# neeharperi/FutureDet

Hardware: AMD Instinct MI355X
Metric: sweeps/sec end-to-end (300k pts, 10-sweep voxel) (higher is better)
Workload: dtype f32

## Files before the change

### futuredet_amd/build.py

```python
import os
import subprocess
import sys

HERE = os.path.dirname(os.path.abspath(__file__))
CSRC = os.path.join(HERE, "csrc")
OUT = os.path.join(HERE, "libfuturedet_hip.so")
SOURCES = ["fd_error.hip", "fd_voxelize.hip", "fd_index.hip", "fd_spconv.hip", "fd_spconv_v2.hip", "fd_spconv_c32.hip", "fd_spconv_f32r.hip", "fd_spconv_bf16.hip", "fd_spconv_bf16win.hip", "fd_densify.hip", "fd_conv2d.hip", "fd_conv2d_f32.hip", "fd_conv2d_wino.hip", "fd_conv2d_wino_pc.hip", "fd_decode.hip", "fd_sweeps.hip", "fd_pillars.hip", "fd_forecast.hip", "fd_deform_conv.hip", "fd_spconv_grad.hip", "fd_targets.hip", "fd_pillars_grad.hip"]
EXTRA = {"fd_decode.hip": ["-ffp-contract=off", "-fno-slp-vectorize"], "fd_sweeps.hip": ["-ffp-contract=off"], "fd_forecast.hip": ["-ffp-contract=off"],
         "fd_voxelize.hip": ["-ffp-contract=off"], "fd_pillars.hip": ["-fno-slp-vectorize"], "fd_pillars_grad.hip": ["-fno-slp-vectorize"],
         "fd_deform_conv.hip": ["-ffp-contract=off", "-fno-slp-vectorize"],
         "fd_targets.hip": ["-ffp-contract=off", "-fno-slp-vectorize"]}


def _hipcc():
    for c in (os.environ.get("HIPCC"), "/opt/rocm/bin/hipcc", "hipcc"):
        if c and (os.path.isfile(c) or c == "hipcc"):
            return c
    return "hipcc"


def needs_build():
    if not os.path.isfile(OUT):
        return True
    t = os.path.getmtime(OUT)
    deps = [os.path.join(CSRC, f) for f in os.listdir(CSRC)] + [os.path.join(HERE, "..", "include", "futuredet_hip.h"), os.path.abspath(__file__)]
    return any(os.path.getmtime(d) > t for d in deps)


def build_locked(force=False, verbose=False):
    import fcntl

    with open(os.path.join(HERE, ".build.lock"), "w") as lk:
        fcntl.flock(lk, fcntl.LOCK_EX)
        try:
            return build(force=force, verbose=verbose)
        finally:
            fcntl.flock(lk, fcntl.LOCK_UN)


def build(force=False, verbose=False):
    if not force and not needs_build():
        return OUT
    objdir = os.path.join(HERE, "csrc", "_obj")
    os.makedirs(objdir, exist_ok=True)
    objs = []
    procs = []
    for src in SOURCES:
        obj = os.path.join(objdir, src.replace(".hip", ".o"))
        cmd = [_hipcc(), "--offload-arch=gfx950", "-O3", "-std=c++17", "-fPIC", "-Wno-unused-value", "-c",
               os.path.join(CSRC, src), "-o", obj] + EXTRA.get(src, [])
        if verbose:
            print(" ".join(cmd))
        procs.append((src, subprocess.Popen(cmd)))
        objs.append(obj)
    for src, p in procs:
        if p.wait() != 0:
            raise RuntimeError("hipcc failed on " + src)
    subprocess.check_call([_hipcc(), "--offload-arch=gfx950", "-shared", "-fPIC", "-o", OUT] + objs)
    return OUT

# ... 4 lines not shown
```

### futuredet_amd/dense_bf16.py

```python
import os

import torch

from . import hip_ops
from .nn_utils import fold_stack


USE_WINOGRAD = not os.environ.get("FD_NO_WINOGRAD")


def granule(dtype):
    return 32 if dtype == torch.bfloat16 else 16


class _Conv(object):
    def __init__(self, w_oihw, bias, stride, relu, dtype):
        self.cout, self.cin, self.ks, _ = w_oihw.shape
        self.stride, self.relu, self.dtype = stride, relu, dtype
        if self.cin % granule(dtype):
            raise ValueError("conv plan: %d input channels are not a multiple of %d" % (self.cin, granule(dtype)))
        self.wpk = hip_ops.pack_conv2d_weight(w_oihw) if dtype == torch.bfloat16 else hip_ops.pack_conv2d_weight_f32(w_oihw)
        self.bias = bias.float().contiguous() if bias is not None else None
        self.fn = hip_ops.conv2d_nhwc_bf16 if dtype == torch.bfloat16 else hip_ops.conv2d_nhwc_f32
        self.wino = (dtype == torch.float32 and self.ks == 3 and stride == 1 and USE_WINOGRAD)
        self.wpk_wino = hip_ops.pack_conv2d_weight_wino(w_oihw) if self.wino else None
        self.choice = {}

    def _run(self, choice, x, out, co_off, kw):
        kind, tile = choice
        if kind == "wino":
            return hip_ops.conv2d_wino_nhwc_f32(x, self.wpk_wino, self.bias, self.cout, self.relu, out=out, co_off=co_off, tile=tile)
        return self.fn(x, self.wpk, self.bias, self.cout, self.ks, self.stride, self.relu, out=out, co_off=co_off, tile=tile, **kw)

    def _pick(self, x, out, co_off, kw):
        key = tuple(x.shape)
        c = self.choice.get(key)
        if c is not None:
            return c
        default = ("wino", 0) if (self.wino and not kw) else ("direct", 0)
        if torch.cuda.is_current_stream_capturing():
            return default
        if out is None:
            out = self._run(default, x, None, co_off, kw)
        if default[0] == "wino":
            cands = [("wino", t) for t in range(0, hip_ops.conv2d_wino_f32_num_tiles() + 1)]
        else:
            cands = [("direct", t) for t in range(0, hip_ops.conv2d_f32_num_tiles() + 1)]
        best, best_ms = default, float("inf")
        for cand in cands:
            try:
                self._run(cand, x, out, co_off, kw)
                ms = float("inf")
                for _ in range(3):
                    e0, e1 = torch.cuda.Event(enable_timing=True), torch.cuda.Event(enable_timing=True)
                    e0.record()
                    for _ in range(4):
                        self._run(cand, x, out, co_off, kw)
                    e1.record()
                    e1.synchronize()
                    ms = min(ms, e0.elapsed_time(e1))
            except hip_ops.FutureDetHipError:
                continue
            if ms < best_ms * 0.98:
                best, best_ms = cand, ms
        self.choice[key] = best
        return best

    def __call__(self, x, out=None, co_off=0, **kw):
        if self.dtype == torch.float32:
            return self._run(self._pick(x, out, co_off, kw), x, out, co_off, kw)
        return self.fn(x, self.wpk, self.bias, self.cout, self.ks, self.stride, self.relu, out=out, co_off=co_off, **kw)


class _GroupedConv(object):

    def __init__(self, wpk, bias, counts, cin_g):
        self.wpk, self.bias, self.counts, self.cin_g = wpk, bias, counts, cin_g

    def __call__(self, x, out=None):
        return hip_ops.conv2d_grouped_nhwc_f32(x, self.wpk, self.bias, self.counts, self.cin_g, relu=False, out=out)


def _convs_from_stack(modules, dtype):
    out = []
    for f in fold_stack(modules, torch.float32, False):
        assert not f.transposed
        assert (f.weight.shape[-1] == 3 and f.padding == 1) or (f.weight.shape[-1] == 1 and f.padding == 0), \
            "only 3x3 pad 1 / 1x1 pad 0 convolutions appear in the RPN / head"
        out.append(_Conv(f.weight, f.bias, f.stride, f.relu, dtype))
    return out


class RPNPlan(object):
    def __init__(self, rpn, dtype=torch.bfloat16):
        self.dtype = dtype
        self.blocks = [_convs_from_stack(b._modules.values(), dtype) for b in rpn.blocks]
        self.start = rpn.first_up
        self.deblocks = []
        for d in rpn.deblocks:
            mods = list(d._modules.values())
            f = fold_stack(mods, torch.float32, False)[0]
            if f.transposed:
                k = f.weight.shape[-1]
                assert f.stride == k and f.padding == 0
                if dtype == torch.float32 and f.weight.shape[1] % 4 == 0 and f.weight.shape[0] % 16 == 0:
                    w = f.weight.permute(2, 3, 1, 0).reshape(-1, f.weight.shape[0])[:, :, None, None].contiguous()
                    self.deblocks.append(("shuffle", k, (hip_ops.pack_conv2d_weight_f32(w), f.bias.float().contiguous(), f.relu), f.weight.shape[1]))
                    continue
                subs = [(_Conv(f.weight[:, :, dy, dx].t().contiguous()[:, :, None, None], f.bias, 1, f.relu, dtype), dy, dx)
                        for dy in range(k) for dx in range(k)]
                self.deblocks.append(("up", k, subs, f.weight.shape[1]))
            elif f.weight.shape[-1] == 1:
                assert f.stride == 1 and f.padding == 0
                self.deblocks.append(("conv", 1, _Conv(f.weight, f.bias, 1, f.relu, dtype), f.weight.shape[0]))
            else:
                k = f.weight.shape[-1]
                assert f.stride == k and f.padding == 0
                w = f.weight.permute(0, 2, 3, 1).reshape(f.weight.shape[0], -1)[:, :, None, None].contiguous()
                self.deblocks.append(("down", k, _Conv(w, f.bias, 1, f.relu, dtype), f.weight.shape[0]))
        self.cout_total = sum(d[3] for d in self.deblocks)

    def __call__(self, x):
        ups = None
        co = 0
        for i, stack in enumerate(self.blocks):
            for conv in stack:
                x = conv(x)
            j = i - self.start
            if j >= 0:
                kind, k, op, cout = self.deblocks[j]
                B, H, W, C = x.shape
                Ho, Wo = (H // k, W // k) if kind == "down" else (H * k, W * k)
                if ups is None:
# ... 26 lines not shown
        if head.bev_map:
            st = fold_stack(head.bev_conv, torch.float32, False)
            g = granule(dtype)
            w0 = st[0].weight
            self.bev_cin = w0.shape[1]
            w0 = torch.cat([w0, torch.zeros((w0.shape[0], (-w0.shape[1]) % g) + tuple(w0.shape[2:]), dtype=w0.dtype, device=w0.device)], dim=1)
            self.bev = [_Conv(w0, st[0].bias, 1, True, dtype)] + [_Conv(f.weight, f.bias, f.stride, f.relu, dtype) for f in st[1:]]
        self.ff = bool(head.forecast_feature)
        self.tasks = []
        self.adapt = []
        self.pre = []
        for ti, task in enumerate(head.tasks):
            if self.ff:
                st = fold_stack(task.forecast_conv, torch.float32, False)
                assert len(st) == 2
                w0 = st[0].weight
                if ti == 0:
                    w0 = torch.cat([w0, torch.zeros_like(w0)], dim=1)
                self.pre.append((_Conv(w0, st[0].bias, 1, True, dtype), _Conv(st[1].weight, st[1].bias, 1, True, dtype)))
            dcn = getattr(task, "task_head", None) is not None
            sep = task.task_head if dcn else task
            names = list(sep.heads)
            stacks = [list(getattr(sep, h)._modules.values()) for h in names]
            if dcn:
                names.append("hm")
                stacks.append(list(task.cls_head._modules.values()))
            firsts, finals = [], []
            for mods in stacks:
                st = fold_stack(mods, torch.float32, False)
                assert len(st) == 2
                firsts.append(st[0])
                finals.append(st[1])
            w1 = torch.cat([f.weight for f in firsts], 0)
            b1 = torch.cat([f.bias for f in firsts], 0)
            adapt = None
            if dcn:
                fc, fr = task.feature_adapt_cls, task.feature_adapt_reg
                adapt = hip_ops.pack_deform_adapt(fc.conv_adaption.weight, fr.conv_adaption.weight, fc.conv_offset.weight, fc.conv_offset.bias,
                                                  fr.conv_offset.weight, fr.conv_offset.bias, dtype == torch.bfloat16)
                cin = w1.shape[1]
                n_hm = firsts[-1].weight.shape[0]
                z = torch.zeros_like(w1)
                w1 = torch.cat([torch.cat([z[:-n_hm], w1[:-n_hm]], 1), torch.cat([w1[-n_hm:], z[-n_hm:]], 1)], 0)
                assert w1.shape[1] == 2 * cin
            hc = firsts[0].weight.shape[0]
            couts = [f.weight.shape[0] for f in finals]
            w2 = torch.zeros((sum(couts), hc * len(names), 3, 3), dtype=torch.float32, device=w1.device)
            o = 0
            for i, f in enumerate(finals):
                w2[o:o + couts[i], i * hc:(i + 1) * hc] = f.weight
                o += couts[i]
            b2 = torch.cat([f.bias for f in finals], 0)
            if dtype == torch.float32 and len(names) <= 8 and max(couts) <= 16 and hc % 16 == 0 and finals[0].weight.shape[-1] == 3:
                wg = torch.zeros((16 * len(names), hc, 3, 3), dtype=torch.float32, device=w1.device)
                bg = torch.zeros((16 * len(names),), dtype=torch.float32, device=w1.device)
                for i, f in enumerate(finals):
                    wg[16 * i:16 * i + couts[i]] = f.weight
                    bg[16 * i:16 * i + couts[i]] = f.bias
                c2 = _GroupedConv(hip_ops.pack_conv2d_weight_f32(wg), bg.contiguous(), list(couts), hc)
            else:
                c2 = _Conv(w2, b2, 1, False, dtype)
            self.tasks.append((_Conv(w1, b1, 1, True, dtype), c2, names, couts))
            self.adapt.append(adapt)

    def __call__(self, x, bev_map=None):
        if self.bev is not None:
            assert bev_map is not None, "this head has a bev_map branch"
            for conv in self.shared:
                x = conv(x)
            B, H, W, _ = x.shape
            y = torch.zeros((B, H, W, self.bev[0].cin), dtype=self.dtype, device=x.device)
            y[..., : self.bev_cin] = bev_map.permute(0, 2, 3, 1)
            for conv in self.bev:
                y = conv(y)
            x = x + y
            return self._tasks(x, None)
        for conv in self.shared[:-1]:
            x = conv(x)
        last = self.shared[-1]
        hc = last.cout
        if self.ff:
            B, H, W, _ = x.shape
            cat = [torch.empty((B, H, W, 2 * hc), dtype=self.dtype, device=x.device) for _ in range(2)]
            cat[0][..., hc:].zero_()
            last(x, out=cat[0], co_off=0)
            cat[1][..., :hc].copy_(cat[0][..., :hc])
        else:
            x = last(x)
            cat = None
        return self._tasks(x, cat)

    def _tasks(self, x, cat):
        hc = self.shared[-1].cout
        if self.ff and cat is None:
            B, H, W, _ = x.shape
            cat = [torch.empty((B, H, W, 2 * hc), dtype=self.dtype, device=x.device) for _ in range(2)]
            cat[0][..., hc:].zero_()
            cat[0][..., :hc].copy_(x)
            cat[1][..., :hc].copy_(x)
        rets = []
        zbuf = None
        for ti, (c1, c2, names, couts) in enumerate(self.tasks):
            d = HeadMaps()
            if self.ff:
                p0, p1 = self.pre[ti]
                x = p1(p0(cat[ti & 1]))
                cat[(ti + 1) & 1][..., hc:].copy_(x)
                d["feats"] = x.permute(0, 3, 1, 2)
            adapt = self.adapt[ti]
            y1 = c1(x if adapt is None else hip_ops.deform_adapt_nhwc(x, adapt[0], adapt[1], adapt[2]))
            uniform = all(tuple(t[3]) == tuple(self.tasks[0][3]) for t in self.tasks)
            if uniform:
# ... 17 lines not shown
```

### futuredet_amd/hip_ops.py

```python
import ctypes
import threading

import numpy as np
import torch

from . import lib as _lib
from .lib import DecodeCfg, FutureDetHipError, MapView, check


_raw_stream = getattr(torch._C, "_cuda_getCurrentRawStream", None)


def _stream():
    if _raw_stream is not None:
        return ctypes.c_void_p(_raw_stream(torch.cuda.current_device()))
    return ctypes.c_void_p(torch.cuda.current_stream().cuda_stream)


def _dev(t, name, dtype=None):
    if not isinstance(t, torch.Tensor) or not t.is_cuda:
        raise FutureDetHipError("%s must be a tensor on the HIP device (got %s); this path has no CPU implementation"
                                % (name, "cpu tensor" if isinstance(t, torch.Tensor) else type(t)))
    if dtype is not None and t.dtype != dtype:
        raise FutureDetHipError("%s must be %s, got %s" % (name, dtype, t.dtype))
# ... 433 lines not shown
    nbytes = L.fd_conv2d_f32_packed_weight_bytes(cout, cin, ks)
    if nbytes == 0:
        raise FutureDetHipError("fd_conv2d_f32: unsupported weight shape %s" % (tuple(w.shape),))
    host = torch.empty((nbytes,), dtype=torch.uint8)
    check(L.fd_conv2d_f32_pack_weight(ctypes.c_void_p(w.data_ptr()), cout, cin, ks, ctypes.c_void_p(host.data_ptr())),
          "fd_conv2d_f32_pack_weight")
    return host.to(dev)


def conv2d_nhwc_f32(x, wpk, bias, cout, ks, stride=1, relu=True, out=None, co_off=0, osy=1, osx=1, ooy=0, oox=0, tile=0):
    L = _lib.load()
    x = _dev(x, "x", torch.float32)
    B, H, W, cin = x.shape
    pad = 1 if ks == 3 else 0
    Ho, Wo = (H + 2 * pad - ks) // stride + 1, (W + 2 * pad - ks) // stride + 1
    if out is None:
        out = torch.empty((B, Ho * osy, Wo * osx, cout), dtype=torch.float32, device=x.device)
    _dev(out, "out", torch.float32)
    check(L.fd_conv2d_nhwc_f32(_p(x), B, H, W, cin, _p(wpk), _p(bias), cout, ks, stride, pad, int(bool(relu)), _p(out),
                               out.shape[3], co_off, osy, osx, ooy, oox, int(tile), _stream()), "fd_conv2d_nhwc_f32")
    return out


def conv2d_f32_num_tiles():
    return int(_lib.load().fd_conv2d_f32_num_tiles())


def conv2d_shuffle_nhwc_f32(x, wpk, bias, cout_sub, k, relu=True, out=None, co_off=0, tile=0):
    L = _lib.load()
    x = _dev(x, "x", torch.float32)
    B, H, W, cin = x.shape
    if out is None:
        out = torch.empty((B, H * k, W * k, cout_sub), dtype=torch.float32, device=x.device)
    _dev(out, "out", torch.float32)
    check(L.fd_conv2d_shuffle_nhwc_f32(_p(x), B, H, W, cin, _p(wpk), _p(bias), int(cout_sub), int(k), int(bool(relu)), _p(out), out.shape[3],
                                       co_off, int(tile), _stream()), "fd_conv2d_shuffle_nhwc_f32")
    return out


def conv2d_grouped_nhwc_f32(x, wpk, bias, counts, cin_g, relu=False, out=None, co_off=0, tile=0):
    L = _lib.load()
    x = _dev(x, "x", torch.float32)
    B, H, W, cin = x.shape
    groups = len(counts)
    assert cin == groups * cin_g
    if out is None:
        out = torch.empty((B, H, W, int(sum(counts))), dtype=torch.float32, device=x.device)
    _dev(out, "out", torch.float32)
    check(L.fd_conv2d_grouped_nhwc_f32(_p(x), B, H, W, groups, int(cin_g), _p(wpk), _p(bias), (ctypes.c_int * groups)(*[int(c) for c in counts]),
                                       int(bool(relu)), _p(out), out.shape[3], co_off, int(tile), _stream()), "fd_conv2d_grouped_nhwc_f32")
    return out


def pack_conv2d_weight_wino(w_oihw):
    L = _lib.load()
    dev = w_oihw.device
    w = w_oihw.detach().to("cpu", torch.float32).contiguous()
    cout, cin, ks, _ = w.shape
    nbytes = L.fd_conv2d_wino_f32_packed_weight_bytes(cout, cin) if ks == 3 else 0
    if nbytes == 0:
        raise FutureDetHipError("fd_conv2d_wino_f32: unsupported weight shape %s" % (tuple(w.shape),))
    host = torch.empty((nbytes,), dtype=torch.uint8)
    check(L.fd_conv2d_wino_f32_pack_weight(ctypes.c_void_p(w.data_ptr()), cout, cin, ctypes.c_void_p(host.data_ptr())),
          "fd_conv2d_wino_f32_pack_weight")
    return host.to(dev)


def conv2d_wino_nhwc_f32(x, wpk, bias, cout, relu=True, out=None, co_off=0, tile=0):
    L = _lib.load()
    x = _dev(x, "x", torch.float32)
    B, H, W, cin = x.shape
    if out is None:
        out = torch.empty((B, H, W, cout), dtype=torch.float32, device=x.device)
    _dev(out, "out", torch.float32)
    check(L.fd_conv2d_wino_nhwc_f32(_p(x), B, H, W, cin, _p(wpk), _p(bias), cout, int(bool(relu)), _p(out), out.shape[3], co_off, int(tile),
                                    _stream()), "fd_conv2d_wino_nhwc_f32")
    return out


def conv2d_wino_f32_num_tiles():
    return int(_lib.load().fd_conv2d_wino_f32_num_tiles())


CIRCLE_PRE_MAX = 4096


def pack_deform_adapt(w_cls, w_reg, off_w_cls, off_b_cls, off_w_reg, off_b_reg, bf16):
    L = _lib.load()
    dev = w_cls.device
    wc = w_cls.detach().to("cpu", torch.float32).contiguous()
    wr = w_reg.detach().to("cpu", torch.float32).contiguous()
    if tuple(wc.shape) != (64, 64, 3, 3) or tuple(wr.shape) != (64, 64, 3, 3):
        raise FutureDetHipError("fd_deform_adapt: conv_adaption weights must be [64, 64, 3, 3], got %s / %s" % (tuple(wc.shape), tuple(wr.shape)))
    host = torch.empty((L.fd_deform_adapt_packed_weight_bytes(int(bool(bf16))),), dtype=torch.uint8)
    check(L.fd_deform_adapt_pack_weight(ctypes.c_void_p(wc.data_ptr()), ctypes.c_void_p(wr.data_ptr()), int(bool(bf16)),
                                        ctypes.c_void_p(host.data_ptr())), "fd_deform_adapt_pack_weight")
    ow = torch.stack([off_w_cls.detach().float().reshape(72, 64), off_w_reg.detach().float().reshape(72, 64)]).contiguous()
    ob = torch.stack([off_b_cls.detach().float().reshape(72), off_b_reg.detach().float().reshape(72)]).contiguous()
    return host.to(dev), ow.to(dev), ob.to(dev)


def deform_adapt_nhwc(x, wpk, off_w=None, off_b=None, offsets=None, out=None):
    L = _lib.load()
    if x.dtype not in (torch.float32, torch.bfloat16):
        raise FutureDetHipError("x must be float32 or bfloat16, got %s" % (x.dtype,))
    x = _dev(x, "x")
# ... 380 lines not shown
```

### futuredet_amd/lib.py

```python
import ctypes
import os

_HERE = os.path.dirname(os.path.abspath(__file__))
LIB_PATH = os.environ.get("FD_LIB_PATH") or os.path.join(_HERE, "libfuturedet_hip.so")
_lib = None

c_void_p = ctypes.c_void_p
c_int = ctypes.c_int
c_i64 = ctypes.c_int64
c_size_t = ctypes.c_size_t
c_float = ctypes.c_float


class MapView(ctypes.Structure):
    _fields_ = [("data", ctypes.c_void_p), ("group_stride", ctypes.c_int64), ("channel_stride", ctypes.c_int64), ("cell_stride", ctypes.c_int64),
                ("dtype", ctypes.c_int)]


ABI_VERSION = 8


class DecodeCfg(ctypes.Structure):
    _fields_ = [("H", c_int), ("W", c_int), ("out_size_factor", c_float), ("voxel_x", c_float), ("voxel_y", c_float),
                ("pc_x", c_float), ("pc_y", c_float), ("score_threshold", c_float), ("center_range", c_float * 6),
# ... 8 lines not shown


class ForecastBuffers(ctypes.Structure):
    _fields_ = [(n, c_void_p) for n in ("center", "quat", "velocity", "size", "fwd_idx", "fwd_ok", "bwd_idx", "bwd_ok", "match_idx", "cv_centers",
                                        "status", "traj_kind", "traj_src", "traj_first", "traj_group", "n_traj")]


class TargetsCfg(ctypes.Structure):
    _fields_ = [("H", c_int), ("W", c_int), ("T", c_int), ("n_max", c_int), ("max_objs", c_int), ("n_sets", c_int), ("n_tasks", c_int),
                ("task_classes", c_int * 16), ("radius_mult", c_int), ("min_radius", c_int), ("out_size_factor", c_float), ("voxel_x", c_float),
                ("voxel_y", c_float), ("pc_x", c_float), ("pc_y", c_float), ("gaussian_overlap", ctypes.c_double)]


SIGNATURES = {
    "fd_abi_version": (c_int, []),
    "fd_last_error": (ctypes.c_char_p, []),
    "fd_tuning_set": (c_int, [ctypes.c_char_p, c_int]),
    "fd_voxelize_workspace_bytes": (c_size_t, [c_i64, c_i64]),
    "fd_voxelize": (c_int, [c_void_p, c_i64, c_void_p, c_int, c_void_p, c_void_p, c_int, c_i64, c_int, c_void_p, c_void_p, c_int,
                            c_void_p, c_int, c_void_p, c_void_p, c_void_p, c_size_t, c_void_p]),
    "fd_index_num_cols": (c_i64, [c_int, c_int, c_int]),
    "fd_index_workspace_bytes": (c_size_t, [c_i64]),
    "fd_index_mark": (c_int, [c_void_p, c_void_p, c_i64, c_int, c_int, c_int, c_int, c_void_p, c_void_p]),
    "fd_index_downsample": (c_int, [c_void_p, c_int, c_int, c_int, c_int, c_void_p, c_void_p, c_void_p, c_void_p, c_void_p]),
    "fd_index_scan": (c_int, [c_void_p, c_i64, c_void_p, c_void_p, c_void_p, c_size_t, c_void_p]),
    "fd_index_coords": (c_int, [c_void_p, c_void_p, c_int, c_int, c_int, c_int, c_void_p, c_void_p]),
    "fd_index_lookup": (c_int, [c_void_p, c_void_p, c_int, c_int, c_int, c_int, c_void_p, c_void_p, c_i64, c_void_p, c_void_p]),
    "fd_rows_permute": (c_int, [c_void_p, c_int, c_void_p, c_void_p, c_i64, c_void_p, c_int, c_int, c_void_p]),
    "fd_rulebook": (c_int, [c_void_p, c_void_p, c_int, c_int, c_int, c_int, c_void_p, c_i64, c_void_p, c_i64, c_int, c_void_p, c_void_p,
                            c_void_p, c_void_p, c_void_p]),
    "fd_spconv_packed_weight_bytes": (c_size_t, [c_int, c_int, c_int, c_int]),
    "fd_spconv_pack_weight": (c_int, [c_void_p, c_int, c_int, c_int, c_int, c_void_p]),
    "fd_spconv_apply": (c_int, [c_void_p, c_i64, c_void_p, c_void_p, c_void_p, c_int, c_void_p, c_i64, c_void_p, c_int, c_int, c_i64,
                                c_void_p, c_i64, c_int, c_int, c_int, c_void_p, c_void_p]),
    "fd_spconv_num_ranges": (c_int, [c_i64, c_int, c_int, c_int]),
    "fd_spconv_wants_balanced_ranges": (c_int, [c_int, c_int, c_int]),
    "fd_spconv_ranges_workspace_bytes": (c_size_t, [c_i64]),
    "fd_spconv_ranges": (c_int, [c_void_p, c_i64, c_int, c_i64, c_void_p, c_int, c_void_p, c_void_p, c_size_t, c_void_p]),
    "fd_densify": (c_int, [c_void_p, c_int, c_int, c_void_p, c_void_p, c_int, c_int, c_int, c_int, c_void_p, c_int, c_i64,
                           c_i64, c_i64, c_i64, c_i64, c_void_p]),
    "fd_conv2d_packed_weight_bytes": (c_size_t, [c_int, c_int, c_int]),
    "fd_conv2d_pack_weight": (c_int, [c_void_p, c_int, c_int, c_int, c_void_p]),
    "fd_conv2d_nhwc_bf16": (c_int, [c_void_p, c_int, c_int, c_int, c_int, c_void_p, c_void_p, c_int, c_int, c_int, c_int, c_int,
                                    c_void_p, c_int, c_int, c_int, c_int, c_int, c_int, c_void_p]),
    "fd_conv2d_f32_packed_weight_bytes": (c_size_t, [c_int, c_int, c_int]),
    "fd_conv2d_f32_pack_weight": (c_int, [c_void_p, c_int, c_int, c_int, c_void_p]),
    "fd_conv2d_f32_num_tiles": (c_int, []),
    "fd_conv2d_nhwc_f32": (c_int, [c_void_p, c_int, c_int, c_int, c_int, c_void_p, c_void_p, c_int, c_int, c_int, c_int, c_int,
                                   c_void_p, c_int, c_int, c_int, c_int, c_int, c_int, c_int, c_void_p]),
    "fd_conv2d_shuffle_nhwc_f32": (c_int, [c_void_p, c_int, c_int, c_int, c_int, c_void_p, c_void_p, c_int, c_int, c_int, c_void_p, c_int, c_int, c_int,
                                           c_void_p]),
    "fd_conv2d_grouped_nhwc_f32": (c_int, [c_void_p, c_int, c_int, c_int, c_int, c_int, c_void_p, c_void_p, c_void_p, c_int, c_void_p, c_int, c_int,
                                           c_int, c_void_p]),
    "fd_conv2d_wino_f32_num_tiles": (c_int, []),
    "fd_conv2d_wino_f32_packed_weight_bytes": (c_size_t, [c_int, c_int]),
    "fd_conv2d_wino_f32_pack_weight": (c_int, [c_void_p, c_int, c_int, c_void_p]),
    "fd_conv2d_wino_nhwc_f32": (c_int, [c_void_p, c_int, c_int, c_int, c_int, c_void_p, c_void_p, c_int, c_int, c_void_p, c_int, c_int, c_int,
                                        c_void_p]),
    "fd_decode_workspace_bytes": (c_size_t, [c_int, ctypes.POINTER(DecodeCfg)]),
    "fd_centerpoint_decode": (c_int, [c_void_p, c_i64, c_void_p, c_i64, c_void_p, c_i64, c_void_p, c_i64, c_void_p, c_i64,
                                      c_int, ctypes.POINTER(DecodeCfg), c_void_p, c_void_p, c_void_p, c_void_p, c_void_p,
                                      c_size_t, c_void_p]),
    "fd_centerpoint_decode_maps": (c_int, [ctypes.POINTER(MapView)] * 5 + [c_int, ctypes.POINTER(DecodeCfg), c_void_p, c_void_p, c_void_p, c_void_p,
                                           c_void_p, c_size_t, c_void_p]),
    "fd_centerpoint_decode_packed": (c_int, [ctypes.POINTER(MapView)] * 6 + [c_int, c_int, ctypes.POINTER(DecodeCfg), c_int, c_void_p, c_void_p, c_void_p,
                                             c_void_p, c_void_p, c_void_p, c_void_p, c_void_p, c_void_p, c_void_p, c_size_t, c_void_p]),
    "fd_assemble_detections": (c_int, [c_void_p, c_void_p, c_void_p, c_void_p, ctypes.POINTER(MapView), c_int, c_int, c_int, c_void_p, c_void_p,
                                       c_void_p, c_void_p, c_void_p, c_void_p]),
    "fd_nms_workspace_bytes": (c_size_t, [c_int]),
    "fd_rotated_nms": (c_int, [c_void_p, c_int, c_float, c_void_p, c_void_p, c_void_p, c_size_t, c_void_p]),
    "fd_boxes_iou_bev": (c_int, [c_void_p, c_int, c_void_p, c_int, c_void_p, c_void_p]),
    "fd_pillar_encode": (c_int, [c_void_p, c_void_p, c_void_p, c_void_p, c_i64, c_int, c_int, c_int, c_float, c_float, c_float,
                                 c_float, c_void_p, c_void_p, c_void_p, c_int, c_void_p, c_void_p, c_void_p, c_int, c_int,
                                 c_void_p, c_int, c_void_p]),
    "fd_pillar_scatter": (c_int, [c_void_p, c_int, c_int, c_int, c_void_p, c_void_p, c_i64, c_int, c_int, c_int, c_void_p, c_int,
                                  c_i64, c_i64, c_i64, c_i64, c_int, c_void_p]),
    "fd_forecast_chains": (c_int, [c_void_p, c_void_p, c_void_p, c_void_p, c_int, c_int, ctypes.c_double, c_void_p, c_void_p,
                                   c_void_p, c_void_p, c_void_p, c_void_p, c_void_p, c_void_p]),
    "fd_det_to_global_boxes": (c_int, [c_void_p, c_int, c_void_p, c_void_p, c_void_p, c_void_p, c_void_p, c_void_p, c_void_p, c_void_p, c_void_p]),
    "fd_forecast_groups": (c_int, [c_void_p, c_int, ctypes.c_double, c_void_p, c_void_p]),
    "fd_forecast_from_detections": (c_int, [c_void_p, c_void_p, c_int, c_int, c_int, c_int, c_void_p, c_void_p, ctypes.c_double, ctypes.c_double,
                                            ctypes.POINTER(ForecastBuffers), c_void_p]),
    "fd_nearest_rows": (c_int, [c_void_p, c_int, c_void_p, c_int, c_int, c_void_p, c_void_p]),
    "fd_index_pyramid": (c_int, [c_void_p, c_void_p, c_i64, c_int, c_int, ctypes.POINTER(IndexLevel), c_void_p, c_void_p, c_size_t,
                                 c_void_p]),
    "fd_index_pyramid_coords": (c_int, [c_int, c_int, ctypes.POINTER(IndexLevel), c_void_p]),
    "fd_rows_place": (c_int, [c_void_p, c_void_p, c_int, c_int, c_int, c_int, c_void_p, c_void_p, c_i64, c_void_p, c_int, c_void_p,
                              c_int, c_int, c_void_p]),
    "fd_sweep_assemble_workspace_bytes": (c_size_t, [c_i64]),
    "fd_sweep_assemble": (c_int, [c_void_p, c_int, c_int, c_i64, c_void_p, c_int, c_float, c_void_p, c_void_p, c_void_p,
                                  c_size_t, c_void_p]),
    "fd_deform_adapt_packed_weight_bytes": (c_size_t, [c_int]),
    "fd_deform_adapt_pack_weight": (c_int, [c_void_p, c_void_p, c_int, c_void_p]),
    "fd_deform_adapt_nhwc": (c_int, [c_void_p, c_int, c_int, c_int, c_int, c_int, c_void_p, c_void_p, c_void_p, c_void_p, c_void_p, c_void_p]),
    "fd_spconv_wgrad_workspace_bytes": (c_size_t, [c_int, c_i64, c_int, c_int]),
    "fd_spconv_wgrad": (c_int, [c_void_p, c_i64, c_void_p, c_void_p, c_i64, c_int, c_i64, c_void_p, c_int, c_int, c_void_p, c_void_p, c_size_t,
                                c_void_p]),
    "fd_rulebook_transpose": (c_int, [c_void_p, c_i64, c_int, c_i64, c_void_p, c_i64, c_void_p, c_i64, c_void_p]),
    "fd_spconv_pack_weight_device": (c_int, [c_void_p, c_int, c_int, c_int, c_int, c_void_p, c_void_p]),
    "fd_dense_gather": (c_int, [c_void_p, c_i64, c_i64, c_i64, c_i64, c_int, c_void_p, c_i64, c_void_p, c_int, c_void_p, c_void_p]),
    "fd_pillar_train_workspace_bytes": (c_size_t, [c_i64, c_int]),
    "fd_pillar_train_forward": (c_int, [c_void_p, c_void_p, c_void_p, c_i64, c_int, c_int, c_int, c_float, c_float, c_float, c_float,
                                        c_void_p, c_void_p, c_void_p, c_int, c_float, c_void_p, c_void_p, c_void_p, c_int, c_float,
                                        c_void_p, c_void_p, c_void_p, c_void_p, c_void_p, c_void_p, c_size_t, c_void_p]),
    "fd_pillar_train_backward": (c_int, [c_void_p, c_void_p, c_void_p, c_i64, c_int, c_int, c_int, c_float, c_float, c_float, c_float,
                                         c_void_p, c_void_p, c_void_p, c_int, c_void_p, c_void_p, c_void_p, c_int, c_void_p,
# ... 35 lines not shown
```

### include/futuredet_hip.h

```cpp
#ifndef FUTUREDET_HIP_H
#define FUTUREDET_HIP_H

#include <stddef.h>
#include <stdint.h>

#ifdef __cplusplus
extern "C" {
#endif

#define FD_OK 0
#define FD_EINVAL (-1)
#define FD_EWORKSPACE (-2)
#define FD_ELAUNCH (-3)

typedef void *fd_stream_t;

int fd_abi_version(void);
const char *fd_last_error(void);
int fd_tuning_set(const char *name, int value);

size_t fd_voxelize_workspace_bytes(int64_t n_points, int64_t max_voxels);
int fd_voxelize(const float *points, int64_t n_points, const int32_t *n_points_dev, int ndim, const float *range6_host,
                const float *voxel_size3_host, int max_points, int64_t max_voxels, int batch_idx,
                float *out_voxels, float *out_mean, int mean_stride, int32_t *out_coors, int coor_cols,
// ... 2 lines not shown

int64_t fd_index_num_cols(int B, int H, int W);
size_t fd_index_workspace_bytes(int64_t num_cols);
int fd_index_mark(const int32_t *coords , const int32_t *n_dev ,
                  int64_t n_max, int B, int D, int H, int W, uint64_t *words, fd_stream_t stream);
int fd_index_downsample(const uint64_t *in_words, int B, int D, int H, int W, const int *ksize3,
                        const int *stride3, const int *pad3, uint64_t *out_words, fd_stream_t stream);
int fd_index_scan(const uint64_t *words, int64_t num_cols, int32_t *prefix, int32_t *n_active_dev,
                  void *workspace, size_t workspace_bytes, fd_stream_t stream);
int fd_index_coords(const uint64_t *words, const int32_t *prefix, int B, int D, int H, int W,
                    int32_t *coords , fd_stream_t stream);
int fd_index_lookup(const uint64_t *words, const int32_t *prefix, int B, int D, int H, int W,
                    const int32_t *coords_in, const int32_t *n_dev, int64_t n_max, int32_t *row_of,
                    fd_stream_t stream);
int fd_rows_permute(const float *src, int c_src, const int32_t *row_of, const int32_t *n_dev, int64_t n_max,
                    void *dst, int c_dst, int dst_bf16, fd_stream_t stream);
int fd_rulebook(const uint64_t *in_words, const int32_t *in_prefix, int B, int Din, int Hin, int Win,
                const int32_t *out_coords, int64_t out_rows, const int32_t *n_out_dev, int64_t nbr_stride, int fill_tail, const int *ksize3,
                const int *stride3, const int *pad3, int32_t *nbr, fd_stream_t stream);

size_t fd_spconv_packed_weight_bytes(int K, int cin, int cout, int dtype);
int fd_spconv_pack_weight(const float *w_kio_host, int K, int cin, int cout, int dtype, void *wpacked_host);
int fd_spconv_apply(const void *in_feats, int64_t n_in, const void *wpacked, const float *bias, const void *residual,
                    int relu, const int32_t *nbr, int64_t nbr_stride, const int32_t *ranges ,
                    int n_ranges, int K, int64_t n_out, const int32_t *n_out_dev ,
                    int64_t n_expected ,
                    int cin, int cout, int dtype, void *out_feats, fd_stream_t stream);
int fd_spconv_num_ranges(int64_t n_out, int cin, int cout, int dtype);
int fd_spconv_wants_balanced_ranges(int cin, int cout, int dtype);
size_t fd_spconv_ranges_workspace_bytes(int64_t n_out);
int fd_spconv_ranges(const int32_t *nbr, int64_t nbr_stride, int K, int64_t n_out, const int32_t *n_out_dev, int n_ranges,
                     int32_t *ranges , void *workspace, size_t workspace_bytes, fd_stream_t stream);

int fd_densify(const void *feats, int c, int dtype, const uint64_t *words, const int32_t *prefix, int B, int D,
               int H, int W, void *out, int out_dtype, int64_t stride_b, int64_t stride_c, int64_t stride_y,
               int64_t stride_x, int64_t n_rows ,
               fd_stream_t stream);

size_t fd_conv2d_packed_weight_bytes(int cout, int cin, int ks);
int fd_conv2d_pack_weight(const float *w_oihw_host, int cout, int cin, int ks, void *wpacked_host);
int fd_conv2d_nhwc_bf16(const void *x, int B, int H, int W, int cin, const void *wpacked, const float *bias, int cout,
                        int ks, int stride, int pad, int relu, void *y, int cout_total, int co_off, int osy, int osx,
                        int ooy, int oox, fd_stream_t stream);
size_t fd_conv2d_f32_packed_weight_bytes(int cout, int cin, int ks);
int fd_conv2d_f32_pack_weight(const float *w_oihw_host, int cout, int cin, int ks, void *wpacked_host);
int fd_conv2d_f32_num_tiles(void);
int fd_conv2d_nhwc_f32(const float *x, int B, int H, int W, int cin, const void *wpacked, const float *bias, int cout, int ks,
                       int stride, int pad, int relu, float *y, int cout_total, int co_off, int osy, int osx, int ooy, int oox,
                       int tile , fd_stream_t stream);
int fd_conv2d_shuffle_nhwc_f32(const float *x, int B, int H, int W, int cin, const void *wpacked, const float *bias, int cout_sub, int k,
                               int relu, float *y, int cout_total, int co_off, int tile, fd_stream_t stream);
int fd_conv2d_grouped_nhwc_f32(const float *x, int B, int H, int W, int groups, int cin_g, const void *wpacked, const float *bias,
                               const int *counts_host, int relu, float *y, int cout_total, int co_off, int tile, fd_stream_t stream);
int fd_conv2d_wino_f32_num_tiles(void);
size_t fd_conv2d_wino_f32_packed_weight_bytes(int cout, int cin);
int fd_conv2d_wino_f32_pack_weight(const float *w_oihw_host, int cout, int cin, void *wpacked_host);
int fd_conv2d_wino_nhwc_f32(const float *x, int B, int H, int W, int cin, const void *wpacked, const float *bias, int cout, int relu,
                            float *y, int cout_total, int co_off, int tile , fd_stream_t stream);

typedef struct fd_decode_cfg {
    int H, W;
    float out_size_factor, voxel_x, voxel_y, pc_x, pc_y;
    float score_threshold;
    float center_range[6];
    float nms_iou_threshold;
    int nms_pre_max, nms_post_max;
    int hm_channels;
    int nms_kind;
    int n_radius;
    float circle_radius[16];
} fd_decode_cfg;

typedef struct fd_map_view {
    const void *data;
    int64_t group_stride, channel_stride, cell_stride;
    int dtype;
} fd_map_view;

size_t fd_decode_workspace_bytes(int G, const fd_decode_cfg *cfg);
int fd_centerpoint_decode_maps(const fd_map_view *hm, const fd_map_view *reg, const fd_map_view *height, const fd_map_view *dim,
                               const fd_map_view *rot, int G, const fd_decode_cfg *cfg_host, float *out_boxes7, float *out_scores,
                               int32_t *out_cell, int32_t *out_count, void *workspace, size_t workspace_bytes, fd_stream_t stream);
int fd_assemble_detections(const float *boxes7, const float *scores, const int32_t *cell, const int32_t *count, const fd_map_view *vel,
                           int B, int post_max, int S, const int32_t *step_group, const int32_t *step_vel_channel,
                           const int32_t *step_label, float *packed, int32_t *counts_out, fd_stream_t stream);
int fd_centerpoint_decode_packed(const fd_map_view *hm, const fd_map_view *reg, const fd_map_view *height, const fd_map_view *dim,
                                 const fd_map_view *rot, const fd_map_view *vel, int G, int B, const fd_decode_cfg *cfg_host, int S,
                                 const int32_t *step_group, const int32_t *step_vel_channel, const int32_t *step_label, float *out_boxes7,
                                 float *out_scores, int32_t *out_cell, int32_t *out_count, float *packed, int32_t *counts_out, void *workspace,
                                 size_t workspace_bytes, fd_stream_t stream);
int fd_centerpoint_decode(const float *hm, int64_t hm_gstride, const float *reg, int64_t reg_gstride,
                          const float *height, int64_t height_gstride, const float *dim, int64_t dim_gstride,
                          const float *rot, int64_t rot_gstride, int G, const fd_decode_cfg *cfg_host,
                          float *out_boxes7, float *out_scores, int32_t *out_cell, int32_t *out_count,
                          void *workspace, size_t workspace_bytes, fd_stream_t stream);

size_t fd_nms_workspace_bytes(int n);
int fd_rotated_nms(const float *boxes7, int n, float thresh, int64_t *keep, int32_t *out_count,
                   void *workspace, size_t workspace_bytes, fd_stream_t stream);
int fd_boxes_iou_bev(const float *a7, int na, const float *b7, int nb, float *out, fd_stream_t stream);

#define FD_SWEEP_HAS_TRANSFORM 1
#define FD_SWEEP_REMOVE_CLOSE 2
typedef struct fd_sweep_desc {
    double m[16];
    int64_t row_begin, row_end;
// ... 107 lines not shown
```

Baseline: 282.1.

## Add tap-sum MFMA kernel for grouped 3x3 head convolutions

```diff
diff --git a/futuredet_amd/build.py b/futuredet_amd/build.py
--- a/futuredet_amd/build.py
+++ b/futuredet_amd/build.py
@@ -5,7 +5,7 @@
 HERE = os.path.dirname(os.path.abspath(__file__))
 CSRC = os.path.join(HERE, "csrc")
 OUT = os.path.join(HERE, "libfuturedet_hip.so")
-SOURCES = ["fd_error.hip", "fd_voxelize.hip", "fd_index.hip", "fd_spconv.hip", "fd_spconv_v2.hip", "fd_spconv_c32.hip", "fd_spconv_f32r.hip", "fd_spconv_bf16.hip", "fd_spconv_bf16win.hip", "fd_densify.hip", "fd_conv2d.hip", "fd_conv2d_f32.hip", "fd_conv2d_wino.hip", "fd_conv2d_wino_pc.hip", "fd_decode.hip", "fd_sweeps.hip", "fd_pillars.hip", "fd_forecast.hip", "fd_deform_conv.hip", "fd_spconv_grad.hip", "fd_targets.hip", "fd_pillars_grad.hip"]
+SOURCES = ["fd_error.hip", "fd_voxelize.hip", "fd_index.hip", "fd_spconv.hip", "fd_spconv_v2.hip", "fd_spconv_c32.hip", "fd_spconv_f32r.hip", "fd_spconv_bf16.hip", "fd_spconv_bf16win.hip", "fd_densify.hip", "fd_conv2d.hip", "fd_conv2d_f32.hip", "fd_conv2d_tapsum_f32.hip", "fd_conv2d_wino.hip", "fd_conv2d_wino_pc.hip", "fd_decode.hip", "fd_sweeps.hip", "fd_pillars.hip", "fd_forecast.hip", "fd_deform_conv.hip", "fd_spconv_grad.hip", "fd_targets.hip", "fd_pillars_grad.hip"]
 EXTRA = {"fd_decode.hip": ["-ffp-contract=off", "-fno-slp-vectorize"], "fd_sweeps.hip": ["-ffp-contract=off"], "fd_forecast.hip": ["-ffp-contract=off"],
          "fd_voxelize.hip": ["-ffp-contract=off"], "fd_pillars.hip": ["-fno-slp-vectorize"], "fd_pillars_grad.hip": ["-fno-slp-vectorize"],
          "fd_deform_conv.hip": ["-ffp-contract=off", "-fno-slp-vectorize"],
diff --git a/futuredet_amd/csrc/fd_conv2d_tapsum_f32.hip b/futuredet_amd/csrc/fd_conv2d_tapsum_f32.hip
--- /dev/null
+++ b/futuredet_amd/csrc/fd_conv2d_tapsum_f32.hip
@@ -0,0 +1,212 @@
+#include "fd_common.h"
+
+namespace {
+
+typedef float f32x4 __attribute__((ext_vector_type(4)));
+
+constexpr int kMaxGroups = 8, kMaxSlices = 4, kMaxCols = 64;
+
+struct TapSumParams {
+    int B, H, W, cin_g, cstride, groups, cout_total, co_off, relu, tiles_x, tiles_y;
+    int buf_floats;
+    int gcnt[kMaxGroups], goff[kMaxGroups], gblk[kMaxGroups];
+    int nblk_total;
+};
+
+inline int blocks_of(int count) { return (9 * count + 15) / 16; }
+
+template <int TH, int TW>
+struct TapSumTile {
+    static constexpr int PH = TH + 2, PW = TW + 2, PP = PH * PW;
+    static constexpr int NPB = (PP + 15) / 16;
+    static constexpr int MBW = (NPB + 3) / 4;
+    static constexpr int PITCH = NPB * 16 + 4;
+    static_assert(TH * TW <= 256, "one thread per output pixel");
+};
+
+template <int TH, int TW>
+__global__ void __launch_bounds__(256) conv3x3_tapsum_f32(const float *__restrict__ x, const float4 *__restrict__ wp, const float *__restrict__ bias,
+                                                          float *__restrict__ y, TapSumParams p) {
+    using T = TapSumTile<TH, TW>;
+    constexpr int PW = T::PW, PP = T::PP, NPB = T::NPB, MBW = T::MBW, PITCH = T::PITCH;
+    extern __shared__ __attribute__((aligned(16))) float smem_p[];
+    __shared__ __attribute__((aligned(16))) float s_bias[64];
+
+    const int tid = threadIdx.x, lane = tid & 63, wave = __builtin_amdgcn_readfirstlane(tid >> 6);
+    const int lm = lane & 15, lq = lane >> 4;
+    int t = blockIdx.x;
+    const int tx = t % p.tiles_x; t /= p.tiles_x;
+    const int ty = t % p.tiles_y; const int b = t / p.tiles_y;
+    const int oy0 = ty * TH, ox0 = tx * TW;
+    const int nsl = p.cin_g >> 4;
+
+    const float *xp[MBW];
+    bool ok[MBW];
+#pragma unroll
+    for (int i = 0; i < MBW; ++i) {
+        const int hp = (wave * MBW + i) * 16 + lm;
+        const int iy = oy0 - 1 + hp / PW, ix = ox0 - 1 + hp % PW;
+        ok[i] = hp < PP && iy >= 0 && iy < p.H && ix >= 0 && ix < p.W;
+        xp[i] = x + (((int64_t)b * p.H + (ok[i] ? iy : 0)) * p.W + (ok[i] ? ix : 0)) * p.cstride + 4 * lq;
+    }
+    float4 xc[MBW][kMaxSlices], xn[MBW][kMaxSlices];
+    auto load_x = [&](int g, float4 (&d)[MBW][kMaxSlices]) {
+#pragma unroll
+        for (int i = 0; i < MBW; ++i)
+#pragma unroll
+            for (int s = 0; s < kMaxSlices; ++s) {
+                d[i][s] = make_float4(0.f, 0.f, 0.f, 0.f);
+                if (ok[i] && s < nsl) d[i][s] = *reinterpret_cast<const float4 *>(xp[i] + g * p.cin_g + 16 * s);
+            }
+    };
+    float4 wc[kMaxSlices], wn[kMaxSlices];
+    auto load_w = [&](int gb, float4 (&d)[kMaxSlices]) {
+        gb = gb < p.nblk_total ? gb : p.nblk_total - 1;
+#pragma unroll
+        for (int s = 0; s < kMaxSlices; ++s) d[s] = wp[((int64_t)gb * nsl + (s < nsl ? s : 0)) * 64 + lane];
+    };
+
+    const int py = tid / TW, px = tid - py * TW;
+    const int oy = oy0 + py, ox = ox0 + px;
+    const bool out_ok = tid < TH * TW && oy < p.H && ox < p.W;
+    float *yp = y + (((int64_t)b * p.H + (out_ok ? oy : 0)) * p.W + (out_ok ? ox : 0)) * p.cout_total + p.co_off;
+    const int sbase = py * PW + px;
+
+    load_x(0, xc);
+    load_w(0, wc);
+    if (tid < p.goff[kMaxGroups - 1] + p.gcnt[kMaxGroups - 1]) s_bias[tid] = bias ? bias[tid] : 0.f;
+    int gb = 0;
+    for (int g = 0; g < p.groups; ++g) {
+        if (g + 1 < p.groups) load_x(g + 1, xn);
+        const int cg = p.gcnt[g], nblk = (9 * cg + 15) >> 4;
+        float *pb = smem_p + (g & 1) * p.buf_floats;
+        for (int nb = 0; nb < nblk; ++nb, ++gb) {
+            load_w(gb + 1, wn);
+            __builtin_amdgcn_sched_barrier(0);
+            f32x4 acc[MBW];
+#pragma unroll
+            for (int i = 0; i < MBW; ++i) acc[i] = f32x4{0.f, 0.f, 0.f, 0.f};
+#pragma unroll
+            for (int s = 0; s < kMaxSlices; ++s) {
+                if (s < nsl) {
+#define FD_KSTEP(C)                                                                                                   \
+    _Pragma("unroll") for (int i = 0; i < MBW; ++i) acc[i] = __builtin_amdgcn_mfma_f32_16x16x4f32(xc[i][s].C, wc[s].C, acc[i], 0, 0, 0);
+                    FD_KSTEP(x) FD_KSTEP(y) FD_KSTEP(z) FD_KSTEP(w)
+#undef FD_KSTEP
+                }
+            }
+            __builtin_amdgcn_sched_barrier(0);
+#pragma unroll
+            for (int i = 0; i < MBW; ++i) {
+                const int blk = wave * MBW + i;
+                if (blk < NPB) *reinterpret_cast<f32x4 *>(pb + (16 * nb + lm) * PITCH + blk * 16 + 4 * lq) = acc[i];
+            }
+#pragma unroll
+            for (int s = 0; s < kMaxSlices; ++s) wc[s] = wn[s];
+        }
+        __syncthreads();
+        if (out_ok) {
+            const float *ps = pb + sbase;
+            for (int c = 0; c < cg; ++c) {
+                float v = s_bias[p.goff[g] + c];
+#pragma unroll
+                for (int tap = 0; tap < 9; ++tap) v += ps[(tap * cg + c) * PITCH + (tap / 3) * PW + tap % 3];
+                if (p.relu) v = fmaxf(v, 0.f);
+                yp[p.goff[g] + c] = v;
+            }
+        }
+        if (g + 1 < p.groups) {
+#pragma unroll
+            for (int i = 0; i < MBW; ++i)
+#pragma unroll
+                for (int s = 0; s < kMaxSlices; ++s) xc[i][s] = xn[i][s];
+        }
+    }
+}
+
+int tapsum_shape(int groups, int cin_g, const int *counts, int *nblk_total, int *nblk_max, int *cout_sum) {
+    if (!counts || groups < 1 || groups > kMaxGroups || cin_g < 16 || cin_g % 16 || cin_g > 16 * kMaxSlices) return 0;
+    int tot = 0, mx = 0, sum = 0;
+    for (int g = 0; g < groups; ++g) {
+        if (counts[g] < 0 || 9 * counts[g] > kMaxCols) return 0;
+        const int nb = blocks_of(counts[g]);
+        tot += nb;
+        mx = nb > mx ? nb : mx;
+        sum += counts[g];
+    }
+    if (tot == 0) return 0;
+    *nblk_total = tot; *nblk_max = mx; *cout_sum = sum;
+    return 1;
+}
+
+}
+
+extern "C" size_t fd_conv2d_tapsum_f32_packed_weight_bytes(int groups, int cin_g, const int *counts_host) {
+    int tot, mx, sum;
+    if (!tapsum_shape(groups, cin_g, counts_host, &tot, &mx, &sum)) return 0;
+    return (size_t)tot * (cin_g / 16) * 64 * 16;
+}
+
+extern "C" int fd_conv2d_tapsum_f32_pack_weight(const float *w, int groups, int cin_g, const int *counts_host, void *dst) {
+    FD_REQUIRE(w && dst, "fd_conv2d_tapsum_f32_pack_weight: null argument");
+    int tot, mx, sum;
+    FD_REQUIRE(tapsum_shape(groups, cin_g, counts_host, &tot, &mx, &sum),
+               "fd_conv2d_tapsum_f32_pack_weight: need 1 <= groups <= 8, cin_g %% 16 == 0, cin_g <= 64 and 9 * counts[g] <= 64");
+    const int nsl = cin_g / 16;
+    float *d = (float *)dst;
+    int gb = 0, goff = 0;
+    for (int g = 0; g < groups; ++g) {
+        const int cg = counts_host[g];
+        for (int nb = 0; nb < blocks_of(cg); ++nb, ++gb)
+            for (int s = 0; s < nsl; ++s)
+                for (int lane = 0; lane < 64; ++lane)
+                    for (int j = 0; j < 4; ++j) {
+                        const int col = 16 * nb + (lane & 15), ci = 16 * s + 4 * (lane >> 4) + j;
+                        float v = 0.f;
+                        if (col < 9 * cg) {
+                            const int tap = col / cg, c = col % cg;
+                            v = w[((int64_t)(goff + c) * cin_g + ci) * 9 + tap];
+                        }
+                        d[(((int64_t)gb * nsl + s) * 64 + lane) * 4 + j] = v;
+                    }
+        goff += cg;
+    }
+    return FD_OK;
+}
+
+extern "C" int fd_conv2d_tapsum_nhwc_f32(const float *x, int B, int H, int W, int groups, int cin_g, const void *wpacked, const float *bias,
+                                         const int *counts_host, int relu, float *y, int cout_total, int co_off, fd_stream_t stream) {
+    FD_REQUIRE(x && wpacked && y && counts_host, "fd_conv2d_tapsum_nhwc_f32: null argument");
+    FD_REQUIRE(B > 0 && H > 0 && W > 0, "fd_conv2d_tapsum_nhwc_f32: bad shape");
+    TapSumParams p;
+    int mx, sum;
+    FD_REQUIRE(tapsum_shape(groups, cin_g, counts_host, &p.nblk_total, &mx, &sum),
+               "fd_conv2d_tapsum_nhwc_f32: need 1 <= groups <= 8, cin_g %% 16 == 0, cin_g <= 64 and 9 * counts[g] <= 64 (fd_conv2d_grouped_nhwc_f32 takes "
+               "the other shapes)");
+    FD_REQUIRE(co_off >= 0 && co_off + sum <= cout_total, "fd_conv2d_tapsum_nhwc_f32: channel window [%d, %d) outside the %d output channels", co_off,
+               co_off + sum, cout_total);
+    FD_REQUIRE(((uintptr_t)x & 15) == 0 && ((uintptr_t)wpacked & 15) == 0, "fd_conv2d_tapsum_nhwc_f32: x and wpacked must be 16-byte aligned");
+    constexpr int TH = 9, TW = 15;
+    using T = TapSumTile<TH, TW>;
+    p.B = B; p.H = H; p.W = W; p.cin_g = cin_g; p.cstride = groups * cin_g; p.groups = groups;
+    p.cout_total = cout_total; p.co_off = co_off; p.relu = relu;
+    p.tiles_x = (W + TW - 1) / TW;
+    p.tiles_y = (H + TH - 1) / TH;
+    p.buf_floats = 16 * mx * T::PITCH;
+    int off = 0, gb = 0;
+    for (int g = 0; g < kMaxGroups; ++g) {
+        const int c = g < groups ? counts_host[g] : 0;
+        p.gcnt[g] = c; p.goff[g] = off; p.gblk[g] = gb;
+        off += c;
+        gb += blocks_of(c);
+    }
+    const int64_t wgs = (int64_t)p.tiles_x * p.tiles_y * B;
+    FD_REQUIRE(wgs <= 0x7fffffff, "fd_conv2d_tapsum_nhwc_f32: too many tiles");
+    const size_t lds = 2 * (size_t)p.buf_floats * sizeof(float);
+    auto kern = conv3x3_tapsum_f32<TH, TW>;
+    static std::atomic<uint64_t> lds_set{0};
+    if (lds > 65536)
+        FD_REQUIRE(fd::ensure_dynamic_lds(reinterpret_cast<const void *>(kern), lds, lds_set), "fd_conv2d_tapsum_nhwc_f32: %zu bytes of LDS refused", lds);
+    hipLaunchKernelGGL(kern, dim3((unsigned)wgs), dim3(256), lds, fd::as_stream(stream), x, (const float4 *)wpacked, bias, y, p);
+    return fd::check_launch("fd_conv2d_tapsum_nhwc_f32");
+}
diff --git a/futuredet_amd/dense_bf16.py b/futuredet_amd/dense_bf16.py
--- a/futuredet_amd/dense_bf16.py
+++ b/futuredet_amd/dense_bf16.py
@@ -7,6 +7,7 @@
 
 
 USE_WINOGRAD = not os.environ.get("FD_NO_WINOGRAD")
+USE_TAPSUM = not os.environ.get("FD_NO_TAPSUM")
 
 
 def granule(dtype):
@@ -74,11 +75,24 @@
 
 class _GroupedConv(object):
 
-    def __init__(self, wpk, bias, counts, cin_g):
-        self.wpk, self.bias, self.counts, self.cin_g = wpk, bias, counts, cin_g
+    def __init__(self, finals, hc):
+        self.counts, self.cin_g = [int(f.weight.shape[0]) for f in finals], int(hc)
+        dev = finals[0].weight.device
+        self.tapsum = USE_TAPSUM and hip_ops.conv2d_tapsum_f32_supported(self.counts, hc)
+        if self.tapsum:
+            self.wpk = hip_ops.pack_conv2d_weight_tapsum_f32(torch.cat([f.weight for f in finals], 0), self.counts)
+            self.bias = torch.cat([f.bias for f in finals], 0).float().contiguous()
+        else:
+            wg = torch.zeros((16 * len(finals), hc, 3, 3), dtype=torch.float32, device=dev)
+            bg = torch.zeros((16 * len(finals),), dtype=torch.float32, device=dev)
+            for i, f in enumerate(finals):
+                wg[16 * i:16 * i + self.counts[i]] = f.weight
+                bg[16 * i:16 * i + self.counts[i]] = f.bias
+            self.wpk, self.bias = hip_ops.pack_conv2d_weight_f32(wg), bg.contiguous()
 
     def __call__(self, x, out=None):
-        return hip_ops.conv2d_grouped_nhwc_f32(x, self.wpk, self.bias, self.counts, self.cin_g, relu=False, out=out)
+        fn = hip_ops.conv2d_tapsum_nhwc_f32 if self.tapsum else hip_ops.conv2d_grouped_nhwc_f32
+        return fn(x, self.wpk, self.bias, self.counts, self.cin_g, relu=False, out=out)
 
 
 def _convs_from_stack(modules, dtype):
@@ -211,12 +225,7 @@
                 o += couts[i]
             b2 = torch.cat([f.bias for f in finals], 0)
             if dtype == torch.float32 and len(names) <= 8 and max(couts) <= 16 and hc % 16 == 0 and finals[0].weight.shape[-1] == 3:
-                wg = torch.zeros((16 * len(names), hc, 3, 3), dtype=torch.float32, device=w1.device)
-                bg = torch.zeros((16 * len(names),), dtype=torch.float32, device=w1.device)
-                for i, f in enumerate(finals):
-                    wg[16 * i:16 * i + couts[i]] = f.weight
-                    bg[16 * i:16 * i + couts[i]] = f.bias
-                c2 = _GroupedConv(hip_ops.pack_conv2d_weight_f32(wg), bg.contiguous(), list(couts), hc)
+                c2 = _GroupedConv(finals, hc)
             else:
                 c2 = _Conv(w2, b2, 1, False, dtype)
             self.tasks.append((_Conv(w1, b1, 1, True, dtype), c2, names, couts))
diff --git a/futuredet_amd/hip_ops.py b/futuredet_amd/hip_ops.py
--- a/futuredet_amd/hip_ops.py
+++ b/futuredet_amd/hip_ops.py
@@ -509,6 +509,41 @@
     return out
 
 
+def conv2d_tapsum_f32_supported(counts, cin_g):
+    n = len(counts)
+    return n >= 1 and int(_lib.load().fd_conv2d_tapsum_f32_packed_weight_bytes(n, int(cin_g), (ctypes.c_int * n)(*[int(c) for c in counts]))) > 0
+
+
+def pack_conv2d_weight_tapsum_f32(w_oihw, counts):
+    L = _lib.load()
+    dev = w_oihw.device
+    w = w_oihw.detach().to("cpu", torch.float32).contiguous()
+    cout, cin_g, ks, ks2 = w.shape
+    n = len(counts)
+    cnt = (ctypes.c_int * max(n, 1))(*[int(c) for c in counts])
+    nbytes = L.fd_conv2d_tapsum_f32_packed_weight_bytes(n, cin_g, cnt) if (ks == 3 and ks2 == 3 and cout == sum(counts)) else 0
+    if nbytes == 0:
+        raise FutureDetHipError("fd_conv2d_tapsum_f32: unsupported weight shape %s for groups %s" % (tuple(w.shape), list(counts)))
+    host = torch.empty((nbytes,), dtype=torch.uint8)
+    check(L.fd_conv2d_tapsum_f32_pack_weight(ctypes.c_void_p(w.data_ptr()), n, cin_g, cnt, ctypes.c_void_p(host.data_ptr())),
+          "fd_conv2d_tapsum_f32_pack_weight")
+    return host.to(dev)
+
+
+def conv2d_tapsum_nhwc_f32(x, wpk, bias, counts, cin_g, relu=False, out=None, co_off=0):
+    L = _lib.load()
+    x = _dev(x, "x", torch.float32)
+    B, H, W, cin = x.shape
+    groups = len(counts)
+    assert cin == groups * cin_g
+    if out is None:
+        out = torch.empty((B, H, W, int(sum(counts))), dtype=torch.float32, device=x.device)
+    _dev(out, "out", torch.float32)
+    check(L.fd_conv2d_tapsum_nhwc_f32(_p(x), B, H, W, groups, int(cin_g), _p(_dev(wpk, "wpk")), _p(bias), (ctypes.c_int * max(groups, 1))(*[int(c) for c in counts]),
+                                      int(bool(relu)), _p(out), out.shape[3], co_off, _stream()), "fd_conv2d_tapsum_nhwc_f32")
+    return out
+
+
 def pack_conv2d_weight_wino(w_oihw):
     L = _lib.load()
     dev = w_oihw.device
diff --git a/futuredet_amd/lib.py b/futuredet_amd/lib.py
--- a/futuredet_amd/lib.py
+++ b/futuredet_amd/lib.py
@@ -84,6 +84,10 @@
                                            c_void_p]),
     "fd_conv2d_grouped_nhwc_f32": (c_int, [c_void_p, c_int, c_int, c_int, c_int, c_int, c_void_p, c_void_p, c_void_p, c_int, c_void_p, c_int, c_int,
                                            c_int, c_void_p]),
+    "fd_conv2d_tapsum_f32_packed_weight_bytes": (c_size_t, [c_int, c_int, c_void_p]),
+    "fd_conv2d_tapsum_f32_pack_weight": (c_int, [c_void_p, c_int, c_int, c_void_p, c_void_p]),
+    "fd_conv2d_tapsum_nhwc_f32": (c_int, [c_void_p, c_int, c_int, c_int, c_int, c_int, c_void_p, c_void_p, c_void_p, c_int, c_void_p, c_int, c_int,
+                                          c_void_p]),
     "fd_conv2d_wino_f32_num_tiles": (c_int, []),
     "fd_conv2d_wino_f32_packed_weight_bytes": (c_size_t, [c_int, c_int]),
     "fd_conv2d_wino_f32_pack_weight": (c_int, [c_void_p, c_int, c_int, c_void_p]),
diff --git a/include/futuredet_hip.h b/include/futuredet_hip.h
--- a/include/futuredet_hip.h
+++ b/include/futuredet_hip.h
@@ -78,6 +78,10 @@
                                int relu, float *y, int cout_total, int co_off, int tile, fd_stream_t stream);
 int fd_conv2d_grouped_nhwc_f32(const float *x, int B, int H, int W, int groups, int cin_g, const void *wpacked, const float *bias,
                                const int *counts_host, int relu, float *y, int cout_total, int co_off, int tile, fd_stream_t stream);
+size_t fd_conv2d_tapsum_f32_packed_weight_bytes(int groups, int cin_g, const int *counts_host);
+int fd_conv2d_tapsum_f32_pack_weight(const float *w_host, int groups, int cin_g, const int *counts_host, void *wpacked_host);
+int fd_conv2d_tapsum_nhwc_f32(const float *x, int B, int H, int W, int groups, int cin_g, const void *wpacked, const float *bias,
+                              const int *counts_host, int relu, float *y, int cout_total, int co_off, fd_stream_t stream);
 int fd_conv2d_wino_f32_num_tiles(void);
 size_t fd_conv2d_wino_f32_packed_weight_bytes(int cout, int cin);
 int fd_conv2d_wino_f32_pack_weight(const float *w_oihw_host, int cout, int cin, void *wpacked_host);
```

Result: no change. 283.5 (median of 6 runs) (+0.5%).
